# Picurit/cutter-vad

Hardware: AMD Instinct MI355X
Metric: 512-sample frames/sec, Silero V5 16kHz, batch=8192 streams per GPU (higher is better)
Workload: dtype f32

## Files before the change

cutter_vad_amd/csrc/silero_v5_t16.hip:

```cpp
#include <hip/hip_runtime.h>
#include <type_traits>
#include <utility>
#include "vad_layout.h"
#include "sm_device.h"
#include "vadk_device.h"

using namespace vadk;

#ifdef VADK_STAMPS
#define STAMP(k)                                                                                   \
    do {                                                                                           \
        if (lane == 0) P.stamps[((size_t)tilei * NWAVES + w) * 32 + (k)] = clock64();          \
    } while (0)
template <class V>
__device__ __forceinline__ void stamp_wait(V v) {
    if constexpr (sizeof(V) == 4) asm volatile("" ::"v"(v) : "memory");
    else if constexpr (sizeof(V) == 32) asm volatile("" ::"v"(v.b.x) : "memory");
    else asm volatile("" ::"v"(v.x) : "memory");
}
#define STAMP_ON(k, v)                                                                             \
    do {                                                                                           \
        if constexpr (!RS) {                                                                       \
            stamp_wait(v);                                                                         \
            STAMP(k);                                                                              \
        }                                                                                          \
    } while (0)
#define STAMP_DRAIN(k)                                                                             \
    do {                                                                                           \
        if constexpr (!RS) {                                                                       \
            asm volatile("s_waitcnt vmcnt(0)" ::: "memory");                                       \
            STAMP(k);                                                                              \
        }                                                                                          \
    } while (0)
#else
#define STAMP(k) do { } while (0)
#define STAMP_ON(k, v) do { } while (0)
#define STAMP_DRAIN(k) do { } while (0)
#endif
using namespace vadk::dev;

namespace {

constexpr int MT16 = 16;
constexpr int QSL = 17;
constexpr int QSD = 16;
constexpr int T_ROW_E0 = 144;
constexpr int T_ROW_E = 168;
constexpr int T_ROW_H = 248;
constexpr int T_ROWS_H = 48;
constexpr int T_ROWS = T_ROW_H + T_ROWS_H;
constexpr int T_ROWS_E1 = 48;
constexpr int T_ROWS_E2 = 24;
static_assert(T_ROW_E0 + 144 <= T_ROWS && T_ROW_E + 32 <= T_ROWS, "enc0's output and enc2's output end inside the activation region");
static_assert(T_ROWS_E1 <= T_ROW_E0, "enc1's planes are written while other waves still read enc0's output");
static_assert(T_ROW_E >= T_ROWS_E1 && T_ROW_E >= 48, "enc2's planes are written while enc1's are read, and read while the x planes are written");
static_assert(T_ROW_E >= T_ROW_E0 && T_ROW_E + T_ROWS_E2 <= T_ROW_H, "enc2's planes lie in enc0's dead output and stay clear of h");
constexpr int T_ROWS_HANDBACK = 64;
static_assert(T_ROW_E0 + T_ROWS_HANDBACK <= T_ROW_H && T_ROWS_H <= T_ROW_E0 && T_ROW_E + T_ROWS_E2 <= T_ROW_H,
              "frames first: the h planes, written behind barrier (4), stay clear of the x planes, enc2's planes and the hand-back rows");
static_assert(T_ROW_H >= T_ROW_E0 && T_ROW_H + T_ROWS_H <= T_ROWS, "frames first: the h planes take the place of enc0's output, dead behind barrier (4)");
constexpr int T_ROWS_DFT = 144;
constexpr int T_EVEN_Q = T_ROWS_DFT * QSD;
constexpr int T_EVEN_ROWS = 96;
static_assert(T_ROWS_DFT == 3 * 4 * 12, "three columns of four plane groups");
static_assert(T_EVEN_Q + T_EVEN_ROWS * QSL <= T_ROW_H * QSD, "the planes and the even operands behind them must end before h");
constexpr int T_FOLD_SINK = 192;
static_assert(96 <= T_FOLD_SINK && T_FOLD_SINK * QSL <= T_ROW_H * QSD, "the 8 kHz sub-model's loader view must end before h");
static_assert(T_ROWS_DFT <= T_ROW_E0 && T_EVEN_Q >= T_ROW_E0 * QSD,
              "the magnitudes (rows 0..143, behind (1b)) take the planes' place; enc0's output (behind (2)) starts where the even operands did");
constexpr int T_LDS_F4 = T_ROWS * QSD + 16 + 12 + 36 + 16 + 96 + 128;
constexpr int T_LSTM_BIAS_BLOCK = 8 + 64 + 64 + 2;
static_assert(T_LDS_F4 * 16 <= 80 * 1024, "stays under half a CU's LDS");
constexpr int T_FLAG_F4 = 2;
static_assert((T_LDS_F4 + T_FLAG_F4) * 16 <= 80 * 1024, "the flags stay under half a CU's LDS");
constexpr int FQ = 129;
constexpr int RS_CH_ROWS = 16;
constexpr int RS_BUF = 4 * RS_CH_ROWS * QSL;
static_assert(2 * RS_BUF <= T_FOLD_SINK * QSL, "resampler staging must fit the loader view");
static_assert((T_LDS_F4 + MT16 * FQ) * 16 <= 160 * 1024, "RS: common layout + F must fit one CU");

__device__ __forceinline__ f32x4 mfma16(f32x4 w, f32x4 a, f32x4 acc) {
    acc = __builtin_amdgcn_mfma_f32_16x16x4f32(w.x, a.x, acc, 0, 0, 0);
    acc = __builtin_amdgcn_mfma_f32_16x16x4f32(w.y, a.y, acc, 0, 0, 0);
    acc = __builtin_amdgcn_mfma_f32_16x16x4f32(w.z, a.z, acc, 0, 0, 0);
    acc = __builtin_amdgcn_mfma_f32_16x16x4f32(w.w, a.w, acc, 0, 0, 0);
    return acc;
}

__device__ __forceinline__ void st_planes(f32x4 *grp, f32x4 xa, f32x4 xb) {
    u32x4 F[3];
    split3_frag(xa, xb, F);
#pragma unroll
    for (int p = 0; p < 3; ++p) grp[4 * p * QSD] = __builtin_bit_cast(f32x4, F[p]);
}
__device__ __forceinline__ void st_planes_half(f32x4 *grp, int half, f32x4 x) {
    u32x2 H[3];
    split3_half(x, H);
#pragma unroll
    for (int p = 0; p < 3; ++p) reinterpret_cast<f32x2 *>(grp + 4 * p * QSD)[half] = __builtin_bit_cast(f32x2, H[p]);
}
#define PL_RD(SRC, s, p) __builtin_bit_cast(u32x4, (SRC)[(12 * (s) + 4 * (p)) * QSD + nq])

constexpr int X3_D = 4;
constexpr int X3_NR = X3_D + 1;

template <class F, int... I>
__device__ __forceinline__ void x3_units(F &&f, std::integer_sequence<int, I...>) {
    (f(std::integral_constant<int, I>{}), ...);
}

}

#define T16_IL(NV, ND)                                                                                          \
    __builtin_amdgcn_sched_group_barrier(0x100, (ND), 0);                                                       \
    _Pragma("unroll") for (int i_ = 0; i_ < (NV); ++i_) {                                                       \
        __builtin_amdgcn_sched_group_barrier(0x008, 4, 0);                                                      \
        __builtin_amdgcn_sched_group_barrier(0x020, 1, 0);                                                      \
    }
#define X3_UNIT(u, U0, B, SRC, EXTRA, FOLD)                                                                     \
    {                                                                                                           \
        constexpr int s_ = (u) >> 3, k_ = (u) & 7;                                                              \
        if constexpr ((u) + X3_D < 32) { X3_LD(B, (u) + X3_D, U0) }                                             \
        if constexpr (k_ == 0 && s_ < 3) { _Pragma("unroll") for (int p_ = 0; p_ < 3; ++p_) N_[p_] = PL_RD(SRC, s_ + 1, p_); } \
        EXTRA(u)                                                                                                \
        G[k_] = mfma_x3(xw[((U0) + (u)) % X3_NR], F_, G[k_]);                                                   \
        if constexpr (k_ == 7) { F_[0] = N_[0]; F_[1] = N_[1]; F_[2] = N_[2]; }                                 \
        if constexpr (!(FOLD(u)) || k_ == 7) SB();                                                              \
    }
#define X3_STEP(s, U0, B, SRC, EXTRA, FOLD)                                                                     \
    X3_UNIT(8 * (s) + 0, U0, B, SRC, EXTRA, FOLD) X3_UNIT(8 * (s) + 1, U0, B, SRC, EXTRA, FOLD)                 \
    X3_UNIT(8 * (s) + 2, U0, B, SRC, EXTRA, FOLD) X3_UNIT(8 * (s) + 3, U0, B, SRC, EXTRA, FOLD)                 \
    X3_UNIT(8 * (s) + 4, U0, B, SRC, EXTRA, FOLD) X3_UNIT(8 * (s) + 5, U0, B, SRC, EXTRA, FOLD)                 \
    X3_UNIT(8 * (s) + 6, U0, B, SRC, EXTRA, FOLD) X3_UNIT(8 * (s) + 7, U0, B, SRC, EXTRA, FOLD)
#define X3_HALF(U0, B, SRC, EXTRA, FOLD)                                                                        \
    {                                                                                                           \
        u32x4 F_[3], N_[3];                                                                                     \
        _Pragma("unroll") for (int p_ = 0; p_ < 3; ++p_) F_[p_] = PL_RD(SRC, 0, p_);                            \
        SB();                                                                                                   \
        X3_STEP(0, U0, B, SRC, EXTRA, FOLD) X3_STEP(1, U0, B, SRC, EXTRA, FOLD)                                 \
        X3_STEP(2, U0, B, SRC, EXTRA, FOLD) X3_STEP(3, U0, B, SRC, EXTRA, FOLD)                                 \
    }
#define X3P_UNIT(v, U0, B, SRC0, SRC1, EXTRA, FOLD)                                                             \
// ... 210 lines not shown
```

cutter_vad_amd/csrc/silero_v5_t16_body.h:

```cpp
#define KP(f) k_##f
    using namespace vadk::v5;
    constexpr bool F32IN = FMT == 0;
    constexpr bool G711 = FMT >= 2;
    static_assert(!RS || F32IN, "resampled frames are float32");
    static_assert(!(RS && K8), "the fused resampler feeds the 16 kHz model");
    static_assert(!SCAN || (!RS && !ONE), "a scan is the frame-loop form on audio in HBM");
    static_assert(CH == 1 || (CH == 2 && SCAN), "two interleaved channels: whole recordings only");
    static_assert(!PAIR || (ONE && !RS && !K8 && !G711 && !SCAN), "paired tiles: one-frame calls of the 16 kHz model, float32 / int16");
    static_assert(!XFIRST || PAIR, "frames first: the paired one-frame kernel (no next frame whose h the cell would hand on)");
    constexpr int QL = K8 ? 8 : 16;
    constexpr int CS = 4 * QL;
    constexpr int PP = K8 ? 24 : 48;
    constexpr int LDS_HALF = T_LDS_F4 + (RS ? MT16 * FQ : 0) + (F32IN ? T_FLAG_F4 : 0);
    static_assert(!PAIR || 2 * LDS_HALF * 16 <= 160 * 1024, "both halves' LDS on one CU");
    __shared__ f32x4 lds[(PAIR ? 2 : 1) * LDS_HALF];
    const int hf = PAIR ? __builtin_amdgcn_readfirstlane((int)threadIdx.x >> 8) : 0;
    f32x4 *const ldsH = PAIR ? lds + hf * LDS_HALF : lds;
    [[maybe_unused]] f32x4 *const ldsO = PAIR ? lds + (1 - hf) * LDS_HALF : lds;
    f32x4 *const RX = ldsH;
    [[maybe_unused]] f32x4 *const REV = ldsH + T_EVEN_Q;
    f32x4 *const RE = ldsH + T_ROW_E * QSD;
    f32x4 *const RP0 = ldsH + T_ROW_E0 * QSD;
    f32x4 *const RH = ldsH + T_ROW_H * QSD;
    float *const headp = reinterpret_cast<float *>(RH + T_ROWS_H * QSD);
    float *const nyqv = headp + 64;
    float *const fcor = nyqv + 48;
    constexpr int FCOR_SINK = 144;
    SmSlot *const smL = reinterpret_cast<SmSlot *>(fcor + 144 + 64);
    f32x4 *const biasL = reinterpret_cast<f32x4 *>(smL + MT16);
    uint8_t *const flagL = reinterpret_cast<uint8_t *>(ldsH + T_LDS_F4 + (RS ? MT16 * FQ : 0));

    const int tid = PAIR ? (int)threadIdx.x & 255 : (int)threadIdx.x;
    const int lane = tid & 63;
    const int w = __builtin_amdgcn_readfirstlane(tid >> 6);
    [[maybe_unused]] const int tilei = PAIR ? 2 * (int)blockIdx.x + hf : (int)blockIdx.x;
    if constexpr (!RS) STAMP(19);
    const int n = lane & 15;
    const int kq = lane >> 4;
    const int nq = kq * QSD + n;
    const int nqL = kq * QSL + n;
    const int vcol = (PAIR ? tilei : (int)blockIdx.x) * MT16 + n;
    int gf = vcol;
    bool live = vcol < KP(n);
    if constexpr (RS) {
        int s0 = R.seg[0].stream0, vs = 0;
#pragma unroll
        for (int k = 1; k < RATE_MAX_SEGS; ++k)
            if (k < R.nseg && vcol >= R.seg[k].vstart) { s0 = R.seg[k].stream0; vs = R.seg[k].vstart; }
        gf = s0 + vcol - vs;
        live = vcol < R.total;
    }
    const int tile0 = (PAIR ? tilei : (int)blockIdx.x) * MT16;
    int slot, ncol = 0;
    uint32_t obase = 0;
    if constexpr (SCAN) {
        const u32x4 it = live ? *reinterpret_cast<const u32x4 *>(k_items + vcol) : u32x4{0u, 0u, 0u, 0u};
        slot = (int)it.x;
        ncol = (int)it.z - S.t0;
        obase = it.w + (uint32_t)S.t0;
    } else {
        slot = live ? (KP(slots) ? KP(slots)[gf] : gf) : 0;
    }
    const __amdgpu_buffer_rsrc_t wrs = __builtin_amdgcn_make_buffer_rsrc(const_cast<float *>(KP(wstream)), 0, (int)KP(wstream_bytes), 0x00020000);
    const int lane16 = lane * 16;
#define WL(blk) ldw(wrs, lane16, (blk))
    const __amdgpu_buffer_rsrc_t wrx = __builtin_amdgcn_make_buffer_rsrc(const_cast<float *>(P.wstream_x), 0, (int)P.wstream_x_bytes, 0x00020000);
#define WX(blk) ldw(wrx, lane16, (blk))
    const __amdgpu_buffer_rsrc_t wry = __builtin_amdgcn_make_buffer_rsrc(const_cast<float *>(P.wstream_y), 0, (int)P.wstream_y_bytes, 0x00020000);
#define WY(blk) ldw(wry, lane16, (blk))
    const int o_stft = (int)P.sect[w][S_STFT], o_nyq = (int)P.sect[w][S_NYQ], o_x0 = (int)P.sect[w][S_ENC0_X3];
    const int o_y1 = (int)P.sect[w][S_ENC1_X3], o_z = 4 * ENC1_X3_BLOCKS + w * ENC23_X3_BLOCKS;
    const int o_l = (int)P.sect[w][S_LSTM], o_x3 = (int)P.sect[w][S_LSTM_X3];
    int T = (ONE || RS) ? 1 : KP(T);
    if constexpr (SCAN) {
        T = min(T, k_items[tile0].nframes - S.t0);
        if (T < 1) return;
    }

    const float thr = P.thresh;
    const int q = tid & (QL - 1);
    const bool q0 = q == 0;
    const int lms = K8 ? (tid >> 3) & 15 : tid >> 4;
    const int lcol = tid >> 7;
    constexpr bool f32in = F32IN;
    constexpr int qsh = (f32in ? 4 : G711 ? 2 : 3) + (CH == 2 ? 1 : 0);
    const float sc = P.fmt == 1 ? 32767.0f : 32768.0f, rsc = 1.0f / sc;
    const __amdgpu_buffer_rsrc_t frs = __builtin_amdgcn_make_buffer_rsrc(
        const_cast<void *>(KP(frames)), 0,
        SCAN ? (int)S.audio_bytes : (int)((unsigned)KP(n) * (unsigned)T * ((f32in ? 2048u : G711 ? 512u : 1024u) >> (K8 ? 1 : 0))), 0x00020000);
    constexpr int X_NT = K8 ? 0 : 2;
    struct XQ2F { u32x4 a, b; };
    using XQ = std::conditional_t<CH == 2, std::conditional_t<f32in, XQ2F, std::conditional_t<G711, u32x2, u32x4>>,
                                  std::conditional_t<G711, uint32_t, u32x4>>;
    auto x_load = [&](int off) -> XQ {
        if constexpr (CH == 2 && f32in)
            return XQ2F{__builtin_amdgcn_raw_buffer_load_b128(frs, off, 0, X_NT), __builtin_amdgcn_raw_buffer_load_b128(frs, off + 16, 0, X_NT)};
        else if constexpr (CH == 2 && G711) return __builtin_amdgcn_raw_buffer_load_b64(frs, off, 0, X_NT);
        else if constexpr (G711) return __builtin_amdgcn_raw_buffer_load_b32(frs, off, 0, X_NT);
        else return __builtin_amdgcn_raw_buffer_load_b128(frs, off, 0, X_NT);
    };
    XQ xa_[4], xb_[4], xc_[4];
    constexpr bool XCARRY = !RS && !K8;
#define X_K0(c) ((XCARRY && (c) > 0) ? 2 : 0)
    f32x4 *const F4 = ldsH + T_LDS_F4;
    uint32_t xq0 = 0;
    [[maybe_unused]] uint32_t xmode = 0;
    if constexpr (SCAN) {
        const int li = tile0 + lms;
        if constexpr (CH == 2) {
            const uint32_t qm = li < KP(n) ? k_items[li].quad0 : 0u;
            xmode = qm >> SCAN_MODE_SHIFT;
            xq0 = (qm & ((1u << SCAN_MODE_SHIFT) - 1u)) + (uint32_t)S.t0 * S.hopq;
        } else {
        xq0 = (li < KP(n) ? k_items[li].quad0 : 0u) + (uint32_t)S.t0 * S.hopq;
        }
    }
#define X_ISSUE(c, XR, tt)                                                                                      \
    if constexpr (RS) {                                                                                         \
        _Pragma("unroll") for (int k = 0; k < 4; ++k)                                                           \
            XR[k] = __builtin_bit_cast(u32x4, F4[(tid >> 4) * FQ + 32 * (c) + q + 16 * k]);                     \
    } else if constexpr (SCAN) {                                                                                \
        const uint32_t fq = xq0 + (uint32_t)(tt) * S.hopq + 32 * (c) + q;                                       \
        _Pragma("unroll") for (int k = X_K0(c); k < 4; ++k)                                                     \
            XR[k] = x_load((int)((fq + 16 * k) << qsh));                                                        \
    } else {                                                                                                    \
        const int fq = ((tile0 + (tid >> 4)) * T + (tt)) * 128 + 32 * (c) + q;                                  \
        _Pragma("unroll") for (int k = X_K0(c); k < 4; ++k)                                                     \
            XR[k] = x_load((fq + 16 * k) << qsh);                                                               \
    }

#define X_ISSUE8(c0, XR, tt)                                                                                    \
    {                                                                                                           \
        const int cc_ = (c0) + lcol < 2 ? (c0) + lcol : 2;                                                      \
        if constexpr (SCAN) {                                                                                   \
            const uint32_t fq = xq0 + (uint32_t)(tt) * S.hopq + 16 * cc_ + q;                                   \
            _Pragma("unroll") for (int k = 0; k < 4; ++k)                                                       \
                XR[k] = x_load((int)((fq + 8 * k) << qsh));                                                     \
        } else {                                                                                                \
        const int fq = ((tile0 + lms) * T + (tt)) * 64 + 16 * cc_ + q;                                          \
        _Pragma("unroll") for (int k = 0; k < 4; ++k)                                                           \
            XR[k] = x_load((fq + 8 * k) << qsh);                                                                \
        }                                                                                                       \
    }

// ... 36 lines not shown
            xl[0] = __builtin_amdgcn_raw_buffer_load_b128(xrs, (sb + s6) * 4, 0, 0);
            xl[1] = __builtin_amdgcn_raw_buffer_load_b128(xrs, (sb + H + s6) * 4, 0, 0);
            xl[2] = __builtin_amdgcn_raw_buffer_load_b128(xrs, (sb + H - s6 - 4) * 4, 0, 0);
            xl[3] = __builtin_amdgcn_raw_buffer_load_b128(xrs, (sb + nn - s6 - 4) * 4, 0, 0);
            const u32x2 a2 = __builtin_amdgcn_raw_buffer_load_b64(xrs, (sb + s6 + 4) * 4, 0, 0);
            const u32x2 c2 = __builtin_amdgcn_raw_buffer_load_b64(xrs, (sb + H + s6 + 4) * 4, 0, 0);
            const u32x2 b2 = __builtin_amdgcn_raw_buffer_load_b64(xrs, (sb + H - s6 - 6) * 4, 0, 0);
            const u32x2 d2 = __builtin_amdgcn_raw_buffer_load_b64(xrs, (sb + nn - s6 - 6) * 4, 0, 0);
            xl[4] = u32x4{a2.x, a2.y, c2.x, c2.y};
            xl[5] = u32x4{b2.x, b2.y, d2.x, d2.y};
        } else {
            xl[0] = __builtin_amdgcn_raw_buffer_load_b128(xrs, (base + qq) * 16, 0, 0);
            xl[1] = __builtin_amdgcn_raw_buffer_load_b128(xrs, (base + qq + (Q >> 1)) * 16, 0, 0);
            xl[2] = __builtin_amdgcn_raw_buffer_load_b128(xrs, (base + (Q >> 1) - qq) * 16, 0, 0);
            xl[3] = __builtin_amdgcn_raw_buffer_load_b128(xrs, (base + (Q >> 1) - qq - 1) * 16, 0, 0);
            xl[4] = __builtin_amdgcn_raw_buffer_load_b128(xrs, (base + (qq == 0 ? 0 : Q - qq)) * 16, 0, 0);
            xl[5] = __builtin_amdgcn_raw_buffer_load_b128(xrs, (base + Q - qq - 1) * 16, 0, 0);
        }
    };
    Part cur = mk_part(0);

    f32x4 hv[2];
    decltype(__builtin_amdgcn_raw_buffer_load_b64(wrs, 0, 0, 0)) bias2;
#define H_STATE_H                                                                                               \
    {                                                                                                           \
        _Pragma("unroll") for (int rt = 0; rt < 2; ++rt)                                                        \
            hv[rt] = *reinterpret_cast<const f32x4 *>(KP(state) + (size_t)slot * 256 + 32 * w + 16 * rt + 4 * kq); \
        SB();                                                                                                   \
        bias2 = __builtin_amdgcn_raw_buffer_load_b64(wrs, lane * 8, (o_l + T_LSTM_BIAS_BLOCK) * 1024, 0);       \
    }
    if constexpr (!XFIRST) H_STATE_H
    const bool sm_thread = (tid < MT16) && live;
    const int sm_slot = slot;
    f32x4 smq[6];
#define H_STATE_SM                                                                                              \
    {                                                                                                           \
        if (tid < MT16) {                                                                                       \
            _Pragma("unroll") for (int k = 0; k < 6; ++k) smq[k] = reinterpret_cast<const f32x4 *>(KP(sm) + slot)[k]; \
        }                                                                                                       \
        SB();                                                                                                   \
    }
    if constexpr (XFIRST) { X_ISSUE(0, xa_, 0) SB(); }
    else H_STATE_SM
    f32x4 xw[X3_NR][3];
    constexpr int NH = PAIR ? 16 : 32, XU_H = K8 ? 0 : (2 * X3_NR - (NH + 4) % X3_NR) % X3_NR, XU_D = XFIRST ? X3_NR - 4 : XU_H + NH;
    static_assert(K8 || (XU_D + 4) % X3_NR == 0, "encoder.0's units follow the DFT's in the ring");
    [[maybe_unused]] const int o_d = 4 * ENC1_X3_BLOCKS + 4 * ENC23_X3_BLOCKS + w * DFT_X3_BLOCKS;
#define X3_LDD(v, slot) X3_LDY(o_d + 3 * (v), slot)
#define X3_LDR(blk, slot) _Pragma("unroll") for (int p_ = 0; p_ < 3; ++p_) xw[(slot) % X3_NR][p_] = WL((blk) + p_);
#define X3_LD(B, u, U0) X3_LDR((B) + 3 * (u), (U0) + (u))
#define X3_LDP(B, v, U0) X3_LDR((B) + 3 * (8 * ((v) >> 2) + 2 * ((v) & 3) + hf), (U0) + (v))
#define X3_LDU(B, u, U0) if constexpr (PAIR) { X3_LDP(B, u, U0) } else { X3_LD(B, u, U0) }
#define X3_LDX(blk, slot) _Pragma("unroll") for (int p_ = 0; p_ < 3; ++p_) xw[(slot) % X3_NR][p_] = WX((blk) + p_);
#define X3_LDY(blk, slot) _Pragma("unroll") for (int p_ = 0; p_ < 3; ++p_) xw[(slot) % X3_NR][p_] = WY((blk) + p_);
#define H_FIRSTX(tt)                                                                                            \
    {                                                                                                           \
        if constexpr (K8) { X_ISSUE8(0, xa_, tt) X_ISSUE8(2, xb_, tt) }                                         \
        else { X_ISSUE(0, xa_, tt) X_ISSUE(1, xb_, tt) }                                                        \
    }
#define H_FIRST(L, tt, WITHX)                                                                                   \
    {                                                                                                           \
        _Pragma("unroll") for (int u_ = 0; u_ < X3_D; ++u_) { X3_LDU((L) + LSTM_X3_HALF_BLOCKS, u_, XU_H) }         \
        if constexpr (WITHX) H_FIRSTX(tt)                                                                       \
        SB();                                                                                                   \
        if constexpr (RS) { X_ISSUE(2, xc_, tt) SB(); }                                                         \
    }
    if constexpr (!RS && !XFIRST) STAMP(29);
    if constexpr (!RS && !XFIRST) H_FIRST(o_x3, 0, K8)
    const f32x4 W1 = ldw(wrs, q * 16, o_nyq), W3 = ldw(wrs, (2 * QL + q) * 16, o_nyq);
    const float w64 = ldw(wrs, QL * 16, o_nyq).x;
    [[maybe_unused]] f32x4 SwF[2];
    if constexpr (XFIRST) {
        X_ISSUE(1, xb_, 0) X_ISSUE(2, xc_, 0)
        SB();
#pragma unroll
        for (int k = 0; k < 2; ++k) SwF[k] = WL(o_stft + 8 + k);
#pragma unroll
        for (int v = 0; v < 4; ++v) { X3_LDD(v, XU_D + v) }
        SB();
        H_STATE_H
        H_STATE_SM
    }
    f32x4 cst[2];
#pragma unroll
    for (int rt = 0; rt < 2; ++rt) cst[rt] = *reinterpret_cast<const f32x4 *>(KP(state) + (size_t)slot * 256 + 128 + 32 * w + 16 * rt + 4 * kq);
    bool chunk0_requested = false;
    if constexpr (RS) {
        if (cur.valid && cur.S.wstream != nullptr && cur.S.n_in == 1536) {
            if (cur.shape == 0) load_chunk(std::integral_constant<int, 0>{}, cur, 0, xlA);
            else load_chunk(std::integral_constant<int, 1>{}, cur, 0, xlA);
            chunk0_requested = true;
        }
    }
    SB();
    if constexpr (XFIRST) STAMP(29);
#define H_TO_LDS                                                                                                \
    {                                                                                                           \
        STAMP_ON(30, hv[1]);                                                                 \
        st_planes(RH + 12 * w * QSD + nq, hv[0], hv[1]);                                                        \
        reinterpret_cast<decltype(bias2) *>(biasL + 32 * w)[lane] = bias2;                                      \
        if (tid < MT16) {                                                                                       \
            _Pragma("unroll") for (int k = 0; k < 6; ++k) reinterpret_cast<f32x4 *>(smL + tid)[k] = smq[k];     \
        }                                                                                                       \
    }
    if constexpr (!XFIRST) {
    STAMP_ON(30, hv[1]);
    st_planes(RH + 12 * w * QSD + nq, hv[0], hv[1]);
    }
    if constexpr (!RS && !K8 && !XFIRST) { SB(); H_FIRSTX(0) SB(); }
    if constexpr (!XFIRST) reinterpret_cast<decltype(bias2) *>(biasL + 32 * w)[lane] = bias2;
    int seg_last = 0;
    if (!XFIRST && tid < MT16) {
#pragma unroll
        for (int k = 0; k < 6; ++k) reinterpret_cast<f32x4 *>(smL + tid)[k] = smq[k];
    }
    const float hb = KP(wstream)[(size_t)P.sect[0][S_HEADB] * BLK_FLOATS];

    if constexpr (RS) {
        float *const Ff = reinterpret_cast<float *>(F4);
        while (cur.valid) {
        const RateSeg S = cur.S;
        const int c0 = cur.c0, c1 = cur.c1, ls0 = cur.ls0;
        auto in_part = [&](int c) { return c >= c0 && c < c1; };
        if (S.wstream == nullptr) {
            const __amdgpu_buffer_rsrc_t xrs =
                __builtin_amdgcn_make_buffer_rsrc(const_cast<float *>(S.in), 0, (int)((unsigned)S.n * 2048u), 0x00020000);
#pragma unroll
            for (int it = 0; it < 8; ++it) {
                const int idx = it * NTHREADS + tid, ms = idx >> 7, qd = idx & 127;
                if (in_part(ms))
                    F4[ms * FQ + qd] = __builtin_bit_cast(f32x4, __builtin_amdgcn_raw_buffer_load_b128(xrs, ((ls0 + ms) * 128 + qd) * 16, 0, 0));
            }
        } else {
          auto run_part = [&](auto p3tag) {
            constexpr int SHAPE = decltype(p3tag)::value;
            constexpr bool P3 = SHAPE == 1 || SHAPE == 2, U2 = SHAPE == 3;
            constexpr int NB = U2 ? 4 : 8;
            constexpr int om = SHAPE;
            const int Q = S.n_in >> 2, Kc = cur.Kc, nchunks = Kc >> 6;
            const float sc0 = 512.0f / (float)S.n_in;
            constexpr float sg3 = om == 1 ? -1.f : 1.f;
            float pA = 0.f;
            const __amdgpu_buffer_rsrc_t ors =
                __builtin_amdgcn_make_buffer_rsrc(const_cast<float *>(S.wstream), 0, (int)S.wstream_bytes, 0x00020000);
            const __amdgpu_buffer_rsrc_t xrs =
                __builtin_amdgcn_make_buffer_rsrc(const_cast<float *>(S.in), 0, (int)((unsigned)S.n * (unsigned)S.n_in * 4u), 0x00020000);
#define OL(blk) ldw(ors, lane16, (blk))
            const int wbase = w * (int)S.wave_blocks;
            if (!chunk0_requested) load_chunk(p3tag, cur, 0, xlA);
            chunk0_requested = false;
            auto store_chunk = [&](int c, int buf, const u32x4 *xl) {
                if constexpr (P3) {
                    const f32x4 A4 = __builtin_bit_cast(f32x4, xl[0]), C4 = __builtin_bit_cast(f32x4, xl[1]);
                    const f32x4 B4 = __builtin_bit_cast(f32x4, xl[2]), D4 = __builtin_bit_cast(f32x4, xl[3]);
                    const f32x4 AC = __builtin_bit_cast(f32x4, xl[4]), BD = __builtin_bit_cast(f32x4, xl[5]);
                    const f32x4 a = f32x4{A4.y, A4.z, AC.x, AC.y}, cc = f32x4{C4.y, C4.z, AC.z, AC.w};
                    const f32x4 b = f32x4{B4.w, B4.z, B4.x, BD.y}, d = f32x4{D4.w, D4.z, D4.x, BD.w};
                    const f32x4 pe = a + cc, me = a - cc, qe = b + d, qo = b - d;
                    f32x4 *dst = lds + buf * RS_BUF + cql * QSL + cms;
                    dst[0] = pe + qe;
                    dst[RS_CH_ROWS * QSL] = pe - qe;
                    dst[2 * RS_CH_ROWS * QSL] = me + qo;
                    dst[3 * RS_CH_ROWS * QSL] = me - qo;
                    const float e0 = A4.x + C4.x + BD.x + BD.z, e3 = A4.w + C4.w + B4.y + D4.y;
                    pA += e0 + sg3 * e3;
                    if (cms >= c0 && cms < c1) {
                        float *o = Ff + cms * (4 * FQ);
                        const int ob = om * 2 * (cql + 16 * c);
// ... 161 lines not shown
                    o[o0 + 4] = y0.z; o[o0 + 260] = y1.z; o[252 - o0] = lo.z; o[508 - o0] = hi.z;
                    o[o0 + 6] = y0.w; o[o0 + 262] = y1.w; o[250 - o0] = lo.w; o[506 - o0] = hi.w;
                }
            } else if constexpr (!P3) {
#pragma unroll
                for (int rt = 0; rt < 2; ++rt) {
                    const int row = 32 * w + 16 * rt + 4 * kq;
                    const f32x4 se = acc[0 + rt], ae = acc[2 + rt], so = acc[4 + rt], ao = acc[6 + rt];
                    const f32x4 pe = se + ae, me = se - ae, pO = so + ao, mO = so - ao;
                    if (in_part(n)) {
                        F4[n * FQ + (row >> 2)] = pe + pO;
                        F4[n * FQ + 64 + (row >> 2)] = pe - pO;
                        const f32x4 lo = me + mO, hi = me - mO;
                        float *o = Ff + n * (4 * FQ);
                        if (row != 0) { o[256 - row] = lo.x; o[512 - row] = hi.x; }
                        o[255 - row] = lo.y; o[511 - row] = hi.y;
                        o[254 - row] = lo.z; o[510 - row] = hi.z;
                        o[253 - row] = lo.w; o[509 - row] = hi.w;
                    }
                }
                headp[rpart * 16 + (tid & 15)] = r128;
                __syncthreads();
                if (tid < MT16 && in_part(tid)) {
                    float e = 0.f, od = 0.f;
#pragma unroll
                    for (int k = 0; k < 8; ++k) { e += headp[k * 16 + tid]; od += headp[(8 + k) * 16 + tid]; }
                    e += mid.x * (xa + xb);
                    od += mid.y * (xa - xb);
                    Ff[tid * (4 * FQ) + 128] = e + od;
                    Ff[tid * (4 * FQ) + 384] = e - od;
                }
            } else {
                headp[rpart * 16 + (tid & 15)] = r128;
                float *const altL = fcor + FCOR_SINK;
                float a = pA;
                a += __shfl_xor(a, 1, 16);
                a += __shfl_xor(a, 2, 16);
                a += __shfl_xor(a, 4, 16);
                a += __shfl_xor(a, 8, 16);
                if (cql == 0) altL[cms] = a * (1.0f / (float)S.n_in);
                __syncthreads();
                const float altv = altL[n];
                const f32x4 altq = f32x4{altv, -altv, altv, -altv};
#pragma unroll
                for (int rt = 0; rt < 2; ++rt) {
                    const int row = 32 * w + 16 * rt + 4 * kq;
                    const f32x4 se = acc[0 + rt], ae = acc[2 + rt], so = acc[4 + rt], ao = acc[6 + rt];
                    const f32x4 pe = se + ae, me = se - ae, pO = so + ao, mO = so - ao;
                    if (in_part(n)) {
                        float *o = Ff + n * (4 * FQ);
                        F4[n * FQ + (row >> 2)] += pe + pO + altq;
                        F4[n * FQ + 64 + (row >> 2)] += pe - pO + altq;
                        const f32x4 lo = me + mO + altq, hi = me - mO + altq;
                        if (row != 0) { o[256 - row] += lo.x; o[512 - row] += hi.x; }
                        o[255 - row] += lo.y; o[511 - row] += hi.y;
                        o[254 - row] += lo.z; o[510 - row] += hi.z;
                        o[253 - row] += lo.w; o[509 - row] += hi.w;
                    }
                }
                if (tid < MT16 && in_part(tid)) {
                    float e = altv, od = 0.f;
#pragma unroll
                    for (int k = 0; k < 8; ++k) { e += headp[k * 16 + tid]; od += headp[(8 + k) * 16 + tid]; }
                    Ff[tid * (4 * FQ) + 128] += e + od;
                    Ff[tid * (4 * FQ) + 384] += e - od;
                }
            }
          };
          if (cur.shape == 0) run_part(std::integral_constant<int, 0>{});
          else if (cur.shape == 1) run_part(std::integral_constant<int, 1>{});
          else if (cur.shape == 2) run_part(std::integral_constant<int, 2>{});
          else run_part(std::integral_constant<int, 3>{});
#undef OL
        }
        __syncthreads();
        cur = mk_part(cur.sk + 1);
        }
    }

    STAMP(0);
    for (int t = 0;;) {
        int ws_stft = o_stft, ws_x0 = o_x0, ws_y1 = o_y1, ws_z = o_z, ws_l = o_l, ws_x3 = o_x3;
        asm volatile("" : "+s"(ws_stft), "+s"(ws_x0), "+s"(ws_y1), "+s"(ws_z), "+s"(ws_l), "+s"(ws_x3));
        f32x4 G[8];
        [[maybe_unused]] f32x4 Gp[4][2];
        {
            [[maybe_unused]] const int wh = ws_x3 + LSTM_X3_HALF_BLOCKS;
            f32x4 xcA, xcB;
            float xm = 0.f;
            auto decode = [&](XQ b) -> f32x4 {
                f32x4 v;
                if constexpr (CH == 2) {
                    f32x4 dl, dr;
                    if constexpr (G711) {
                        dl = g711_quad<FMT == 3>(__builtin_amdgcn_perm(b.y, b.x, 0x06040200u));
                        dr = g711_quad<FMT == 3>(__builtin_amdgcn_perm(b.y, b.x, 0x07050301u));
                    } else if constexpr (!f32in) {
                        dl = f32x4{i16_div((int)(short)(b.x & 0xffffu), sc, rsc), i16_div((int)(short)(b.y & 0xffffu), sc, rsc),
                                   i16_div((int)(short)(b.z & 0xffffu), sc, rsc), i16_div((int)(short)(b.w & 0xffffu), sc, rsc)};
                        dr = f32x4{i16_div((int)(short)(b.x >> 16), sc, rsc), i16_div((int)(short)(b.y >> 16), sc, rsc),
                                   i16_div((int)(short)(b.z >> 16), sc, rsc), i16_div((int)(short)(b.w >> 16), sc, rsc)};
                    } else {
                        dl = __builtin_bit_cast(f32x4, u32x4{b.a.x, b.a.z, b.b.x, b.b.z});
                        dr = __builtin_bit_cast(f32x4, u32x4{b.a.y, b.a.w, b.b.y, b.b.w});
                    }
                    const bool right = xmode == 1u, mix = xmode >= 2u;
                    const f32x4 mx = pk::mul(pk::add(dl, dr), f32x4{0.5f, 0.5f, 0.5f, 0.5f});
                    v.x = mix ? mx.x : right ? dr.x : dl.x;
                    v.y = mix ? mx.y : right ? dr.y : dl.y;
                    v.z = mix ? mx.z : right ? dr.z : dl.z;
                    v.w = mix ? mx.w : right ? dr.w : dl.w;
                    if constexpr (f32in) xm = absmax4(xm, v);
                } else if constexpr (G711) {
                    v = g711_quad<FMT == 3>(b);
                } else if constexpr (!f32in) {
                    const int s0 = (int)(short)(b.x & 0xffffu), s1 = (int)(short)(b.x >> 16);
                    const int s2 = (int)(short)(b.y & 0xffffu), s3 = (int)(short)(b.y >> 16);
                    v = f32x4{i16_div(s0, sc, rsc), i16_div(s1, sc, rsc), i16_div(s2, sc, rsc), i16_div(s3, sc, rsc)};
                } else {
                    v = __builtin_bit_cast(f32x4, b);
                    xm = absmax4(xm, v);
                }
                return gate4(v, thr);
            };
#define X_FLAG                                                                                                  \
    if constexpr (f32in) {                                                                                      \
        const unsigned long long b_ = __builtin_amdgcn_ballot_w64(nonfinite(xm));                               \
        flagL[(K8 ? 16 * lcol : 0) + lms] = (uint8_t)(((b_ >> (lane & (64 - QL))) & ((1ull << QL) - 1)) != 0);   \
    }
            auto mirror = [](float v) -> float {
                return __builtin_bit_cast(float, __builtin_amdgcn_mov_dpp(__builtin_bit_cast(int, v), K8 ? 0x141 : 0x140, 0xf, 0xf, true));
            };
            auto shr1 = [&](float edge, float v) -> float {
                const float r = __builtin_bit_cast(float, __builtin_amdgcn_update_dpp(__builtin_bit_cast(int, edge), __builtin_bit_cast(int, v), 0x111, 0xf, 0xf, false));
                return (K8 && q0) ? edge : r;
            };
            auto shl8 = [](float v) -> float {
                return __builtin_bit_cast(float, __builtin_amdgcn_mov_dpp(__builtin_bit_cast(int, v), 0x108, 0xf, 0xf, true));
            };
            [[maybe_unused]] auto ror8hi = [](float lo, float hi) -> float {
                return __builtin_bit_cast(float, __builtin_amdgcn_update_dpp(__builtin_bit_cast(int, lo), __builtin_bit_cast(int, hi), 0x128, 0xf, 0xc, false));
            };
            [[maybe_unused]] const int fold_og = (12 * (q >> 3) + (q & 3)) * QSD + (lms ^ ((q & 3) | ((q >> 3) << 2)));
#define X_FOLD(c, XR, NEXT)                                                                                     \
    {                                                                                                           \
        _Pragma("clang fp contract(off)")                                                                       \
        const int ms = lms;                                                                                     \
        STAMP_ON(20 + (NEXT), XR[3]);                                                                           \
        f32x4 xA, xB;                                                                                           \
        if constexpr (XCARRY && (NEXT)) { xA = xcA; xB = xcB; }                                                 \
        else { xA = decode(XR[0]); xB = decode(XR[1]); }                                                        \
        const f32x4 xC = decode(XR[2]), xD = decode(XR[3]);                                                     \
        if constexpr (XCARRY) { xcA = xC; xcB = xD; }                                                           \
        const float mBx = mirror(xB.x), mDx = mirror(xD.x);                                                     \
        const f32x4 y1 = pk::mul(xA, W1), y3 = pk::mul(xC, W3);                                                 \
        const f32x4 y2 = pk::mul(f32x4{shr1(xC.x, mBx), mirror(xB.w), mirror(xB.z), mirror(xB.y)}, W3);         \
        const f32x4 y4 = pk::mul(f32x4{shr1(0.f, mDx), mirror(xD.w), mirror(xD.z), mirror(xD.y)}, W1);          \
        const f32x4 s14 = pk::add(y1, y4), d14 = pk::sub(y1, y4), s23 = pk::add(y2, y3), d23 = pk::sub(y2, y3); \
        f32x4 pe = pk::add(s14, s23), po = pk::sub(s14, s23), qe = pk::sub(d14, d23), qo = pk::add(d14, d23);   \
        {                                                                                                       \
            pe.x = q0 ? 0.f : pe.x; po.x = q0 ? 0.f : po.x; qe.x = q0 ? 0.f : qe.x; qo.x = q0 ? 0.f : qo.x;        \
            const float y64 = xB.x * w64, y192 = xD.x * w64;                                                    \
            const int fo = q0 ? (c) * 48 + ms : FCOR_SINK + lane;                                               \
            fcor[fo] = y3.x;                                                                                    \
            fcor[fo + (q0 ? 16 : 0)] = y64 + y192;                                                              \
            fcor[fo + (q0 ? 32 : 0)] = y64 - y192;                                                              \
        }                                                                                                       \
// ... 402 lines not shown
            x3_units([&](auto uc_) {
                constexpr int v_ = decltype(uc_)::value;
                if constexpr (v_ < NU3) { X3_LDY(E3_BLK(v_), XU_3 + v_) }
                else { X3_LDN(v_ - NU3) }
                if constexpr (v_ + 1 < NU2) {
#pragma unroll
                    for (int p_ = 0; p_ < 3; ++p_) F_[(v_ + 1) & 1][p_] = PL_RD(RX, v_ + 1, p_);
                }
                acc = mfma_x3(xw[(XU_2 + v_) % X3_NR], F_[v_ & 1], acc);
                SB();
            }, std::make_integer_sequence<int, NU2>{});
            st_planes_half(RE + 12 * (w >> 1) * QSD + nq, w & 1, relu4(acc));
        }
        STAMP(9);
        __syncthreads();
        STAMP(10);

        if constexpr (PAIR) {
            f32x4 acc[2] = {e3b[0], e3b[0]};
#define E3P_SRC(st) ((st) ? ldsO + T_ROW_E * QSD : RE)
            u32x4 F_[2][2][3];
#pragma unroll
            for (int st = 0; st < 2; ++st)
#pragma unroll
                for (int p_ = 0; p_ < 3; ++p_) F_[st][0][p_] = PL_RD(E3P_SRC(st), 0, p_);
            SB();
            x3_units([&](auto uc_) {
                constexpr int v_ = decltype(uc_)::value;
                X3_LDN(v_ + X3_D - NU3)
                if constexpr (v_ == 0) {
#pragma unroll
                    for (int st = 0; st < 2; ++st)
#pragma unroll
                        for (int p_ = 0; p_ < 3; ++p_) F_[st][1][p_] = PL_RD(E3P_SRC(st), 1, p_);
                }
#pragma unroll
                for (int st = 0; st < 2; ++st) acc[st] = mfma_x3(xw[(XU_3 + v_) % X3_NR], F_[st][v_], acc[st]);
                SB();
            }, std::make_integer_sequence<int, NU3>{});
#undef E3P_SRC
#pragma unroll
            for (int st = 0; st < 2; ++st) st_planes_half((st ? ldsO : ldsH) + 12 * w * QSD + nq, hf, relu4(acc[st]));
            if constexpr (XFIRST) {
                STAMP(31);
                const f32x4 *const bq = biasL + 32 * w + kq;
#pragma unroll
                for (int k = 0; k < 4; ++k) Gp[k][0] = Gp[k][1] = bq[k * 8 + hf * 4];
#define HX_EXTRA(v) if constexpr ((v) + X3_D >= NH) { X3_LDP(ws_x3, (v) + X3_D - NH, XU_L) }
#define HX_FOLDREGION(v) false
                X3P_HALF(XU_R, (ws_x3 + LSTM_X3_HALF_BLOCKS), RH, (ldsO + T_ROW_H * QSD), HX_EXTRA, HX_FOLDREGION)
#undef HX_EXTRA
#undef HX_FOLDREGION
                STAMP(26);
            }
        } else {
            f32x4 acc[2] = {e3b[0], e3b[1]};
            u32x4 F_[2][3];
#pragma unroll
            for (int p_ = 0; p_ < 3; ++p_) F_[0][p_] = PL_RD(RE, 0, p_);
            SB();
            x3_units([&](auto uc_) {
                constexpr int v_ = decltype(uc_)::value, s_ = v_ >> 1, rt_ = v_ & 1;
                X3_LDU(ws_x3, v_, XU_L)
                if constexpr (v_ == 0) {
#pragma unroll
                    for (int p_ = 0; p_ < 3; ++p_) F_[1][p_] = PL_RD(RE, 1, p_);
                }
                acc[rt_] = mfma_x3(xw[(XU_3 + v_) % X3_NR], F_[s_], acc[rt_]);
                SB();
            }, std::make_integer_sequence<int, NU3>{});
            st_planes(RX + 12 * w * QSD + nq, relu4(acc[0]), relu4(acc[1]));
        }
#undef E3_BLK
#undef X3_LDN
        STAMP(11);
        __syncthreads();
        STAMP(12);

        {
            const int ws = ws_l + 8;
            f32x4 hw[2];
#define L_EXTRA(u) if constexpr ((u) == 24) { hw[0] = WL(ws + 128); hw[1] = WL(ws + 129); }
#define L_FOLDREGION(u) false
#define LP_EXTRA(v) if constexpr ((v) == 12) { hw[0] = WL(ws + 128); hw[1] = WL(ws + 129); }
            if constexpr (PAIR) {
                X3P_HALF(XU_L, ws_x3, RX, ldsO, LP_EXTRA, L_FOLDREGION)
                f32x4 *const hb = ldsO + (T_ROW_E0 + 16 * w) * QSD + nq;
#pragma unroll
                for (int k = 0; k < 4; ++k) hb[4 * k * QSD] = Gp[k][1];
            } else {
            X3_HALF(XU_L, ws_x3, RX, L_EXTRA, L_FOLDREGION)
            }
#undef LP_EXTRA
#undef L_EXTRA
#undef L_FOLDREGION
            STAMP(18);
            STAMP(13);
            __syncthreads();
            STAMP(14);
            if constexpr (PAIR) {
                const f32x4 *const hb = ldsH + (T_ROW_E0 + 16 * w) * QSD + nq;
#pragma unroll
                for (int k = 0; k < 4; ++k) {
                    const f32x4 o = hb[4 * k * QSD];
                    G[2 * k] = hf ? o : Gp[k][0];
                    G[2 * k + 1] = hf ? Gp[k][0] : o;
                }
            }
            f32x4 part4 = f32x4{0.f, 0.f, 0.f, 0.f};
            const bool rej = f32in && (K8 ? (flagL[n] | flagL[16 + n]) : flagL[n]) != 0;
            const bool bad = SCAN ? (rej || t >= ncol) : rej;
            f32x4 hq[2];
#pragma unroll
            for (int rt = 0; rt < 2; ++rt) {
                const f32x4 i4 = G[0 + rt], f4 = G[2 + rt], g4 = G[4 + rt], o4 = G[6 + rt], c4 = cst[rt], hwv = hw[rt];
                f32x4 cn = pk::fma(pk::sigmoid4(f4), c4, pk::mul(pk::sigmoid4(i4), pk::tanh4(g4)));
                f32x4 hn = pk::mul(pk::sigmoid4(o4), pk::tanh4(cn));
                part4 = pk::fma(hwv, relu4(hn), part4);
                if constexpr ((f32in || SCAN) && !ONE && !RS) {
                    hn = bad ? hv[rt] : hn;
                    cn = bad ? c4 : cn;
                    hv[rt] = hn;
                }
                hq[rt] = hn;
                if (t == T - 1 && live && !((ONE || RS) && bad)) {
                    *reinterpret_cast<f32x4 *>(KP(state) + (size_t)slot * 256 + 32 * w + 16 * rt + 4 * kq) = hn;
                    *reinterpret_cast<f32x4 *>(KP(state) + (size_t)slot * 256 + 128 + 32 * w + 16 * rt + 4 * kq) = cn;
                }
                cst[rt] = cn;
            }
            if constexpr (!ONE && !RS) st_planes(RH + 12 * w * QSD + nq, hq[0], hq[1]);
            float part_ = (part4.x + part4.y) + (part4.z + part4.w);
            part_ += __shfl_xor(part_, 16);
            part_ += __shfl_xor(part_, 32);
            if (kq == 0) headp[w * 16 + n] = part_;
        }
        __syncthreads();
        STAMP(15);

        if (tid < MT16) {
            const float z = hb + ((headp[tid] + headp[16 + tid]) + (headp[32 + tid] + headp[48 + tid]));
            const float p = fminf(sigmoidf_(z), 1.0f);
            if (sm_thread) {
                const bool bad = f32in && (K8 ? (flagL[tid] | flagL[16 + tid]) : flagL[tid]) != 0;
                if constexpr (SCAN) {
                    SmSlot sm = smL[tid];
                    if (t < ncol) {
                        const size_t o = (size_t)obase + (size_t)t;
                        int seg = 0;
                        const int ev = bad ? EV_REJECTED : sm_step(sm, p, &seg);
                        P.probs[o] = bad ? __builtin_nanf("") : p;
                        if (P.events) P.events[o] = (uint8_t)ev;
                        if (P.seg_frames) P.seg_frames[o] = (ev & 2) ? seg : 0;
                    }
                    if (t == T - 1) KP(sm)[sm_slot] = sm;
                    else smL[tid] = sm;
                } else {
                P.probs[(size_t)gf * T + t] = bad ? __builtin_nanf("") : p;
                SmSlot sm = smL[tid];
                int seg = 0;
                const int ev = bad ? EV_REJECTED : sm_step(sm, p, &seg);
                if (t == T - 1) { if (!((ONE || RS) && bad)) KP(sm)[sm_slot] = sm; }
                else smL[tid] = sm;
                if (ev & 2) seg_last = seg;
                if (P.events) P.events[(size_t)gf * T + t] = (uint8_t)ev;
                }
            }
        }
        if (++t >= T) break;
        if constexpr (!RS) H_FIRST(ws_x3, t, true)
    }
#undef H_TO_LDS
#undef H_STATE_SM
#undef H_STATE_H
#undef H_FIRST
#undef H_FIRSTX
#undef X3_LDU
#undef X3_LDP
#undef X3_LD
#undef X3_LDR
#undef X3_LDX
#undef X3_LDD
#undef X3_LDY
#undef WY
#undef WX
#undef X_ISSUE
#undef X_K0
#undef WL
    if constexpr (!SCAN) { if (sm_thread && P.seg_frames) P.seg_frames[gf] = seg_last; }
    if constexpr (!RS) STAMP(27);
    STAMP_DRAIN(28);
#undef KP
```

Baseline: 268.7 million.

## Compute LSTM cell in place per half and exchange only head partials in paired tiles

In the paired one-frame kernel, each half now finishes the LSTM cell for its own hidden slice on both tiles' streams, using the gate partials it already holds. This replaces the old step where all gate partials were handed back through LDS and recomputed per tile. Only the head-weight products are exchanged through a small LDS region, and the original post-LSTM barrier is folded into that exchange. Each half also loads the cell state and writes h/c for both tiles, which needs the other tile's slot and liveness computed up front. The aim is to cut LDS traffic and register pressure, at the cost of an extra barrier inside the exchange and more intricate cross-half indexing.

```diff
diff --git a/cutter_vad_amd/csrc/silero_v5_t16.hip b/cutter_vad_amd/csrc/silero_v5_t16.hip
--- a/cutter_vad_amd/csrc/silero_v5_t16.hip
+++ b/cutter_vad_amd/csrc/silero_v5_t16.hip
@@ -55,9 +55,11 @@
 static_assert(T_ROWS_E1 <= T_ROW_E0, "enc1's planes are written while other waves still read enc0's output");
 static_assert(T_ROW_E >= T_ROWS_E1 && T_ROW_E >= 48, "enc2's planes are written while enc1's are read, and read while the x planes are written");
 static_assert(T_ROW_E >= T_ROW_E0 && T_ROW_E + T_ROWS_E2 <= T_ROW_H, "enc2's planes lie in enc0's dead output and stay clear of h");
-constexpr int T_ROWS_HANDBACK = 64;
-static_assert(T_ROW_E0 + T_ROWS_HANDBACK <= T_ROW_H && T_ROWS_H <= T_ROW_E0 && T_ROW_E + T_ROWS_E2 <= T_ROW_H,
-              "frames first: the h planes, written behind barrier (4), stay clear of the x planes, enc2's planes and the hand-back rows");
+constexpr int T_ROWS_HEADX = 32;
+static_assert(T_ROWS_H <= T_ROW_E0 && T_ROW_E0 + T_ROWS_HEADX <= T_ROW_H,
+              "the head exchange rows lie above the x planes, which the input half of other waves is still reading, and below the h planes");
+static_assert(T_ROW_E0 + T_ROWS_HEADX <= T_ROW_H && T_ROWS_H <= T_ROW_E0 && T_ROW_E + T_ROWS_E2 <= T_ROW_H,
+              "frames first: the h planes, written behind barrier (4), stay clear of the x planes, enc2's planes and the head exchange rows");
 static_assert(T_ROW_H >= T_ROW_E0 && T_ROW_H + T_ROWS_H <= T_ROWS, "frames first: the h planes take the place of enc0's output, dead behind barrier (4)");
 constexpr int T_ROWS_DFT = 144;
 constexpr int T_EVEN_Q = T_ROWS_DFT * QSD;
diff --git a/cutter_vad_amd/csrc/silero_v5_t16_body.h b/cutter_vad_amd/csrc/silero_v5_t16_body.h
--- a/cutter_vad_amd/csrc/silero_v5_t16_body.h
+++ b/cutter_vad_amd/csrc/silero_v5_t16_body.h
@@ -60,6 +60,14 @@
         obase = it.w + (uint32_t)S.t0;
     } else {
         slot = live ? (KP(slots) ? KP(slots)[gf] : gf) : 0;
+    }
+    [[maybe_unused]] bool live_o = false;
+    [[maybe_unused]] int slot_o = 0;
+    if constexpr (PAIR) {
+        const int vcol_o = (tilei ^ 1) * MT16 + n;
+        live_o = vcol_o < KP(n);
+        slot_o = live_o ? vcol_o : 0;
+        if (KP(slots)) slot_o = KP(slots)[slot_o];
     }
     const __amdgpu_buffer_rsrc_t wrs = __builtin_amdgcn_make_buffer_rsrc(const_cast<float *>(KP(wstream)), 0, (int)KP(wstream_bytes), 0x00020000);
     const int lane16 = lane * 16;
@@ -262,8 +270,13 @@
         H_STATE_SM
     }
     f32x4 cst[2];
+    if constexpr (PAIR) {
+        cst[0] = *reinterpret_cast<const f32x4 *>(KP(state) + (size_t)slot * 256 + 128 + 32 * w + 16 * hf + 4 * kq);
+        cst[1] = *reinterpret_cast<const f32x4 *>(KP(state) + (size_t)slot_o * 256 + 128 + 32 * w + 16 * hf + 4 * kq);
+    } else {
 #pragma unroll
     for (int rt = 0; rt < 2; ++rt) cst[rt] = *reinterpret_cast<const f32x4 *>(KP(state) + (size_t)slot * 256 + 128 + 32 * w + 16 * rt + 4 * kq);
+    }
     bool chunk0_requested = false;
     if constexpr (RS) {
         if (cur.valid && cur.S.wstream != nullptr && cur.S.n_in == 1536) {
@@ -591,7 +604,7 @@
     for (int t = 0;;) {
         int ws_stft = o_stft, ws_x0 = o_x0, ws_y1 = o_y1, ws_z = o_z, ws_l = o_l, ws_x3 = o_x3;
         asm volatile("" : "+s"(ws_stft), "+s"(ws_x0), "+s"(ws_y1), "+s"(ws_z), "+s"(ws_l), "+s"(ws_x3));
-        f32x4 G[8];
+        [[maybe_unused]] f32x4 G[8];
         [[maybe_unused]] f32x4 Gp[4][2];
         {
             [[maybe_unused]] const int wh = ws_x3 + LSTM_X3_HALF_BLOCKS;
@@ -1160,12 +1173,9 @@
             f32x4 hw[2];
 #define L_EXTRA(u) if constexpr ((u) == 24) { hw[0] = WL(ws + 128); hw[1] = WL(ws + 129); }
 #define L_FOLDREGION(u) false
-#define LP_EXTRA(v) if constexpr ((v) == 12) { hw[0] = WL(ws + 128); hw[1] = WL(ws + 129); }
+#define LP_EXTRA(v) if constexpr ((v) == 12) { hw[0] = WL(ws + 128 + hf); }
             if constexpr (PAIR) {
                 X3P_HALF(XU_L, ws_x3, RX, ldsO, LP_EXTRA, L_FOLDREGION)
-                f32x4 *const hb = ldsO + (T_ROW_E0 + 16 * w) * QSD + nq;
-#pragma unroll
-                for (int k = 0; k < 4; ++k) hb[4 * k * QSD] = Gp[k][1];
             } else {
             X3_HALF(XU_L, ws_x3, RX, L_EXTRA, L_FOLDREGION)
             }
@@ -1174,17 +1184,50 @@
 #undef L_FOLDREGION
             STAMP(18);
             STAMP(13);
+            if constexpr (PAIR) {
+                static_assert(!PAIR || ONE, "no barrier (7): nothing rewrites the h planes");
+                const uint8_t *const flagO = reinterpret_cast<const uint8_t *>(ldsO + T_LDS_F4);
+                float *const headpO = reinterpret_cast<float *>(ldsO + (T_ROW_H + T_ROWS_H) * QSD);
+                f32x4 *const hx = lds + (T_ROW_E0 + 8 * w) * QSD + nq;
+                f32x4 hr[2];
+                int sl[2] = {slot, slot_o};
+                asm volatile("" : "+v"(sl[0]), "+v"(sl[1]));
+                asm volatile("" ::"v"(hw[0]) : "memory");
+#pragma unroll
+                for (int st = 0; st < 2; ++st) {
+                    const f32x4 i4 = Gp[0][st], f4 = Gp[1][st], g4 = Gp[2][st], o4 = Gp[3][st], c4 = cst[st];
+                    const f32x4 cn = pk::fma(pk::sigmoid4(f4), c4, pk::mul(pk::sigmoid4(i4), pk::tanh4(g4)));
+                    const f32x4 hn = pk::mul(pk::sigmoid4(o4), pk::tanh4(cn));
+                    hr[st] = relu4(hn);
+                    const bool bad = f32in && (st ? flagO[n] : flagL[n]) != 0;
+                    if ((st ? live_o : live) && !bad) {
+                        float *const sp = KP(state) + (size_t)sl[st] * 256 + 32 * w + 16 * hf + 4 * kq;
+                        *reinterpret_cast<f32x4 *>(sp) = hn;
+                        *reinterpret_cast<f32x4 *>(sp + 128) = cn;
+                    }
+                }
+                if (hf == 0) {
+#pragma unroll
+                    for (int st = 0; st < 2; ++st) hx[4 * st * QSD] = pk::fma(hw[0], hr[st], f32x4{0.f, 0.f, 0.f, 0.f});
+                }
+                STAMP(14);
+                __syncthreads();
+                STAMP(15);
+                if (hf != 0) {
+#pragma unroll
+                    for (int st = 0; st < 2; ++st) {
+                        const f32x4 part4 = pk::fma(hw[0], hr[st], hx[4 * (1 - st) * QSD]);
+                        float part_ = (part4.x + part4.y) + (part4.z + part4.w);
+                        part_ += __builtin_bit_cast(float, __builtin_amdgcn_ds_bpermute((lane ^ 16) << 2, __builtin_bit_cast(int, part_)));
+                        part_ += __builtin_bit_cast(float, __builtin_amdgcn_ds_bpermute((lane ^ 32) << 2, __builtin_bit_cast(int, part_)));
+                        if (kq == 0) (st ? headpO : headp)[w * 16 + n] = part_;
+                    }
+                }
+                __syncthreads();
+                STAMP(16);
+            } else {
             __syncthreads();
             STAMP(14);
-            if constexpr (PAIR) {
-                const f32x4 *const hb = ldsH + (T_ROW_E0 + 16 * w) * QSD + nq;
-#pragma unroll
-                for (int k = 0; k < 4; ++k) {
-                    const f32x4 o = hb[4 * k * QSD];
-                    G[2 * k] = hf ? o : Gp[k][0];
-                    G[2 * k + 1] = hf ? Gp[k][0] : o;
-                }
-            }
             f32x4 part4 = f32x4{0.f, 0.f, 0.f, 0.f};
             const bool rej = f32in && (K8 ? (flagL[n] | flagL[16 + n]) : flagL[n]) != 0;
             const bool bad = SCAN ? (rej || t >= ncol) : rej;
@@ -1212,9 +1255,12 @@
             part_ += __shfl_xor(part_, 16);
             part_ += __shfl_xor(part_, 32);
             if (kq == 0) headp[w * 16 + n] = part_;
-        }
+            }
+        }
+        if constexpr (!PAIR) {
         __syncthreads();
         STAMP(15);
+        }
 
         if (tid < MT16) {
             const float z = hb + ((headp[tid] + headp[16 + tid]) + (headp[32 + tid] + headp[48 + tid]));
```

After: 271.7 million, median of 6. +1.1%, better.
